# Ameek94/BOBE

Measured on AMD Instinct MI355X. Metric: GP fit+acquisition cycles/sec at N=4096 d=8, 65536 cands; Cholesky GF/s, higher is better.
Workload: dtype f64

## Files before the change

bobe_amd/_lib.py:

```python
from __future__ import annotations

import ctypes as C
import os
from typing import Optional

import numpy as np

_HERE = os.path.dirname(os.path.abspath(__file__))
LIB_PATH = os.path.join(_HERE, "libbobe_gp.so")

BOBE_OK = 0
BOBE_NOT_PD = 1
MAX_MLL_SLOTS = 8
PROF = {"potf2": 1, "trsm": 2, "syrk": 3, "trtri": 4, "lauum": 5, "trimul": 6, "cross": 7, "kxx": 8, "crossvv": 9, "kxc": 10}

c_double_p = C.POINTER(C.c_double)
c_int64_p = C.POINTER(C.c_int64)


class BobeLibraryError(RuntimeError):
    pass


SIGNATURES = [
# ... 59 lines not shown
    ("bobe_mgpu_world", C.c_int, []),
    ("bobe_mgpu_rank", C.c_int, []),
    ("bobe_mgpu_finalize", None, []),
    ("bobe_mgpu_wip_sweep", C.c_int, [C.c_void_p, C.c_void_p, C.c_int64, C.c_int64, C.c_void_p, C.c_int64, C.c_double,
                                      C.c_void_p, C.c_void_p, C.c_void_p, C.c_void_p,
                                      c_int64_p, c_double_p, c_int64_p, c_double_p]),
    ("bobe_mgpu_best_fit", C.c_int, [C.c_double, C.c_void_p, C.c_int, c_double_p, C.c_void_p]),
    ("bobe_gp_npoints", C.c_int64, [C.c_void_p]),
    ("bobe_debug_gemm", C.c_int, [C.c_int, C.c_int, C.c_int, C.c_int64, C.c_int64, C.c_int64, C.c_void_p, C.c_int64,
                                  C.c_void_p, C.c_int64, C.c_void_p, C.c_int64]),
    ("bobe_debug_kinv", C.c_int, [C.c_void_p, C.c_void_p]),
    ("bobe_debug_linv", C.c_int, [C.c_void_p, C.c_void_p]),
    ("bobe_debug_time_potrf", C.c_int, [C.c_void_p, C.c_int, c_double_p]),
    ("bobe_debug_time_potrf_batch", C.c_int, [C.c_void_p, C.c_int, C.c_int, c_double_p]),
    ("bobe_debug_time_potrf_lockstep", C.c_int, [C.c_void_p, C.c_int, C.c_int, c_double_p]),
    ("bobe_gp_set_chunk", C.c_int, [C.c_void_p, C.c_int64]),
    ("bobe_gp_profile_select", C.c_int, [C.c_void_p, C.c_int]),
    ("bobe_gp_profile_read", C.c_int, [C.c_void_p, c_double_p, c_int64_p]),
    ("bobe_debug_mfma_peak", C.c_int, [C.c_int, C.c_int, c_double_p]),
    ("bobe_debug_wave_sums", C.c_int, [C.c_int, C.c_int, C.c_void_p, C.c_void_p]),
]

_lib: Optional[C.CDLL] = None


def load() -> C.CDLL:
    global _lib
    if _lib is not None:
        return _lib
    if not os.path.exists(LIB_PATH):
# ... 42 lines not shown
```

bobe_amd/csrc/gp_abi.hip:

```cpp
#include "gp_handle.hpp"

#include "kernels_common.hpp"

#include <dlfcn.h>
#include <rccl/rccl.h>

using namespace bobe;

namespace bobe {
thread_local std::string g_err;
}

namespace {

template <int LA, int LB>
__global__ __launch_bounds__(256, 2) void k_debug_gemm(const double* __restrict__ A, int64_t lda,
                                                    const double* __restrict__ B, int64_t ldb, double* __restrict__ C,
                                                    int64_t ldc, int64_t K) {
  extern __shared__ double smem[];
  v4d acc[4][4];
  acc_zero(acc);
  gemm_tile<LA, LB>(acc, A, lda, (int64_t)blockIdx.y * TILE, B, ldb, (int64_t)blockIdx.x * TILE, 0, K, smem);
  store_tile(acc, C, ldc, (int64_t)blockIdx.y * TILE, (int64_t)blockIdx.x * TILE, 1.0, 0.0);
}
// ... 513 lines not shown
  API_BEGIN
  NEED(g && ms && reps >= 1 && B >= 1 && B <= BOBE_MAX_MLL_SLOTS, "bad argument");
  *ms = g->time_potrf_batch(B, reps);
  return BOBE_OK;
  API_END
}

int bobe_debug_time_potrf_lockstep(bobe_gp_t* g, int B, int reps, double* ms) {
  API_BEGIN
  NEED(g && ms && reps >= 1 && B >= 1 && B <= BOBE_MAX_MLL_SLOTS, "bad argument");
  *ms = g->time_potrf_lockstep(B, reps);
  return BOBE_OK;
  API_END
}

int bobe_gp_profile_select(bobe_gp_t* g, int tag) {
  API_BEGIN
  NEED(g, "gp is NULL");
  g->use();
  g->sync();
  g->prof_tag = tag;
  g->prof_used = 0;
  return BOBE_OK;
  API_END
}

int bobe_gp_profile_read(bobe_gp_t* g, double* total_ms, int64_t* launches) {
  API_BEGIN
  NEED(g && total_ms && launches, "NULL argument");
  g->use();
// ... 306 lines not shown
```

bobe_amd/csrc/gp_consumers.hip:

```cpp
#include "gp_handle.hpp"

#include "consumer_kernels.hpp"

using namespace bobe;

namespace bobe {
void configure_consumer_kernels() {
  static bool done[64] = {false};
  int dev = 0;
  HIPCHK(hipGetDevice(&dev));
  if (dev < 0 || dev >= 64 || done[dev]) return;
#define BIG(KE, DC)                                         \
  allow_big_lds((k_hmc_run<KE, DC>), CHAIN_LDS_BYTES);      \
  allow_big_lds((k_rwalk<KE, DC>), CHAIN_LDS_BYTES)
  BIG(0, 8); BIG(0, 16); BIG(0, 32); BIG(1, 8); BIG(1, 16); BIG(1, 32);
#undef BIG
  done[dev] = true;
}
}

void bobe_gp::set_gate(const double* sv, int64_t n_sv, const double* dual, double intercept, double gamma, double threshold,
                       double minus_inf) {
  use();
  sync();
// ... 289 lines not shown
      for (auto& v : dg) v += hk.noise;
      HIPCHK(hipMemcpy2D(out, (size_t)(nB + 1) * sizeof(double), dg.data(), sizeof(double), sizeof(double), (size_t)nA,
                         hipMemcpyHostToDevice));
    }
  }
}

void bobe_gp::clone_from(bobe_gp& src) {
  if (this == &src) return;
  if (d != src.d || kern != src.kern || device != src.device)
    throw Err(BOBE_ERR_ARG, "clone needs handles of the same kernel, dimension and device");
  if (!src.have_data) throw Err(BOBE_ERR_STATE, "source holds no data");
  src.use();
  src.sync();
  sync();
  N = src.N;
  hyp = src.hyp;
  pivot_ulp = src.pivot_ulp;
  refine_kappa = src.refine_kappa;
  solve_block = src.solve_block;
  solve_panel = src.solve_panel;
  solve_chunk = src.solve_chunk;
  refine_v = src.factored && src.refine_v;
  if (Np != src.Np) {
    Np = src.Np;
    nb = src.nb;
    alloc_for_n();
  }
  const size_t mat = (size_t)src.Np * src.Np * sizeof(double), vec = (size_t)src.Np * sizeof(double);
  X.ensure((size_t)(src.Np + TILE) * src.d * sizeof(double));
// ... 66 lines not shown
```

bobe_amd/csrc/gp_factor.hip:

```cpp
#include "gp_handle.hpp"

#include <chrono>

#include "chol_kernels.hpp"

using namespace bobe;

namespace bobe {

constexpr int SYRK32_BK = 128, SYRK64_BK = 16;
constexpr int SYRK32_SMEM = gemm_smem_doubles_exact<KC, KC, 32, 32, SYRK32_BK>() * 8 / 2;
constexpr int SYRK64_SMEM = gemm_smem_doubles_exact<KC, KC, 64, 64, SYRK64_BK>() * 8;

void configure_factor_kernels() {
  static bool done[64] = {false};
  int dev = 0;
  HIPCHK(hipGetDevice(&dev));
  if (dev < 0 || dev >= 64 || done[dev]) return;
  allow_big_lds(k_potf2<true>, POTF2_SMEM_BYTES);
  allow_big_lds(k_potf2<false>, POTF2_SMEM_BYTES);
  allow_big_lds(k_trti_diag, POTF2_SMEM_BYTES);
  allow_big_lds(k_trsm_panel, TRSM_SMEM_BYTES);
  allow_big_lds((k_chol_panel<false, 3>), POTF2_SMEM_BYTES);
  allow_big_lds((k_chol_panel<false, 4>), POTF2_SMEM_BYTES);
// ... 13 lines not shown
  allow_big_lds(k_lauum_grad<0, 32, 64>, GEMM64_SMEM_BYTES);
  allow_big_lds(k_lauum_grad<1, 8, 64>, GEMM64_SMEM_BYTES);
  allow_big_lds(k_lauum_grad<1, 16, 64>, GEMM64_SMEM_BYTES);
  allow_big_lds(k_lauum_grad<1, 32, 64>, GEMM64_SMEM_BYTES);
  allow_big_lds(k_lauum_grad<0, 8, 128>, GEMM_SMEM_BYTES);
  allow_big_lds(k_lauum_grad<0, 16, 128>, GEMM_SMEM_BYTES);
  allow_big_lds(k_lauum_grad<0, 32, 128>, GEMM_SMEM_BYTES);
  allow_big_lds(k_lauum_grad<1, 8, 128>, GEMM_SMEM_BYTES);
  allow_big_lds(k_lauum_grad<1, 16, 128>, GEMM_SMEM_BYTES);
  allow_big_lds(k_lauum_grad<1, 32, 128>, GEMM_SMEM_BYTES);
  done[dev] = true;
}

const Tuning& tuning() {
  static Tuning t = [] {
    Tuning v{512, 600, 300, 1, BOBE_MAX_MLL_SLOTS, 2048, 1, 1, false, false};
    auto geti = [](const char* name, int& dst) {
      const char* e = std::getenv(name);
      if (e) dst = std::atoi(e);
      return e != nullptr;
    };
    geti("BOBE_SYRK32_BELOW", v.syrk32_below);
    geti("BOBE_TRTRI64", v.trtri64_below);
    geti("BOBE_PAIR_MIN", v.pair_min);
    geti("BOBE_LOCKSTEP_MIN_N", v.lockstep_min_n);
    v.mll_slots_set = geti("BOBE_MLL_SLOTS", v.mll_slots);
    geti("BOBE_GRAPH_MAX_N", v.graph_max_n);
    geti("BOBE_XCD_SHARES", v.xcd_shares);
    geti("BOBE_FILL", v.fill);
    v.trace = std::getenv("BOBE_TRACE") != nullptr;
    return v;
  }();
  return t;
}

double default_refine_kappa() {
  static const double v = [] {
    const char* e = std::getenv("BOBE_REFINE_KAPPA");
    return e ? std::atof(e) : 1e6;
  }();
  return v;
}

int default_solve_block() {
  static const int v = [] {
// ... 79 lines not shown
  alpha.ensure(vec);
  w.ensure(vec);
  alpha2.ensure(vec);
  w2.ensure(vec);
  XsT.ensure((size_t)d * vec);
  XsT2.ensure((size_t)d * vec);
  const int64_t pw = Np > chunk ? Np : chunk;
  part.ensure((size_t)nb * pw * sizeof(double));
  gpart.ensure((size_t)(2 * nb) * (2 * nb + 1) / 2 * (MAX_D + 1) * sizeof(double));
  res.ensure(128 * sizeof(double));
  info.ensure(sizeof(int));
  flags.ensure((size_t)nb * sizeof(int));
  diag.ensure((size_t)nb * TILE * TILE * sizeof(double));
  build_probs();
  build_plans();
}

void bobe_gp::scale(const double* in, int64_t n, int64_t npad, const Hyper& h, double* out, int64_t ldo,
                    const Hyper* hdev, int B, int64_t bsO, int* info_reset) {
  hipLaunchKernelGGL(k_scale_coords, dim3((unsigned)((npad + 255) / 256), (unsigned)B), dim3(256), 0, stream, in, n, npad,
                     h, out, ldo, hdev, bsO, info_reset);
  LAUNCH_CHECK();
}

#define KM_LAUNCH(KE, SQ, DC, grid, ...)                                                                 \
  do {                                                                                                   \
    if (h.d == DC)                                                                                       \
      hipLaunchKernelGGL((k_kernel_matrix<KE, SQ, DC, true>), grid, dim3(256), 0, stream, __VA_ARGS__);  \
    else                                                                                                 \
      hipLaunchKernelGGL((k_kernel_matrix<KE, SQ, DC, false>), grid, dim3(256), 0, stream, __VA_ARGS__); \
// ... 402 lines not shown
  factor_into(h, XsT2.d(), A2.d(), Linv2.d(), w2.d(), alpha2.d(), hdev);
  if (want_grad) {
    const int dcap = d <= 8 ? 8 : (d <= 16 ? 16 : 32);
    const int ntiles = lauum(h, Linv2.d(), alpha2.d(), XsT2.d(), nullptr, dcap, hdev, nullptr, 1, 0, 0, 0, 0, Tmp.d(), 0);
    hipLaunchKernelGGL(k_mll_grad_reduce, dim3(d + 2), dim3(256), 0, stream, (const double*)gpart.d(), ntiles, dcap + 1, d,
                       dcap, res.d(), (const double*)w2.d(), (const double*)A2.d(), Np, Np, (const int*)info.p);
  } else {
    hipLaunchKernelGGL(k_mll_terms, dim3(1), dim3(256), 0, stream, (const double*)w2.d(), (const double*)A2.d(), Np, Np,
                       res.d(), (int64_t)0, (int64_t)0, (int64_t)0, (const int*)info.p);
  }
  LAUNCH_CHECK();
  HIPCHK(hipMemcpyAsync(h_res, res.p, 102 * sizeof(double), hipMemcpyDeviceToHost, stream));
}

void bobe_gp::mll_enqueue(const Hyper& h, bool want_grad) {
  const Tuning& tu = tuning();
  h_res[110] = pivot_floor(h);
  if (!in_slot || N > tu.graph_max_n || prof_tag != 0) {
    mll_enqueue_body(h, want_grad, nullptr);
    return;
  }
  if (!eg.h_hyp) HIPCHK(hipHostMalloc(reinterpret_cast<void**>(&eg.h_hyp), sizeof(Hyper), hipHostMallocDefault));
  eg.hyp_dev.ensure(sizeof(Hyper));
  const int w = want_grad ? 1 : 0;
  const std::array<const void*, 16> sig = eval_signature();
  if (!eg.exec[w] || eg.sig[w] != sig) {
    if (eg.exec[w]) {
      (void)hipGraphExecDestroy(eg.exec[w]);
      eg.exec[w] = nullptr;
    }
// ... 10 lines not shown
    const hipError_t ie = hipGraphInstantiate(&eg.exec[w], graph, nullptr, nullptr, 0);
    (void)hipGraphDestroy(graph);
    if (ie != hipSuccess) {
      eg.exec[w] = nullptr;
      HIPCHK(ie);
    }
    eg.sig[w] = sig;
  }
  *eg.h_hyp = h;
  HIPCHK(hipGraphLaunch(eg.exec[w], stream));
}

int bobe_gp::slot_collect(Slot& sl, double* mll, double* grad) {
  HIPCHK(hipStreamSynchronize(sl.stream));
  const double* hr = sl.h_res;
  int inf;
  std::memcpy(&inf, hr + 100, sizeof(int));
  if (inf != 0x7f7f7f7f || !pivots_resolved(hr[101], hr[110])) {
    *mll = std::nan("");
    if (grad)
      for (int j = 0; j <= d; ++j) grad[j] = std::nan("");
    g_err = not_pd_text(inf, hr[101]);
    return BOBE_NOT_PD;
  }
  *mll = -0.5 * hr[0] - hr[1] - 0.5 * (double)N * std::log(2.0 * M_PI);
  if (grad)
    for (int j = 0; j <= d; ++j) grad[j] = hr[2 + j];
  return BOBE_OK;
}

int bobe_gp::mll_collect(double* mll, double* grad) {
  sync();
  int inf;
  std::memcpy(&inf, h_res + 100, sizeof(int));
  if (inf != 0x7f7f7f7f || !pivots_resolved(h_res[101], h_res[110])) {
    *mll = std::nan("");
    if (grad)
      for (int j = 0; j <= d; ++j) grad[j] = std::nan("");
    g_err = not_pd_text(inf, h_res[101]);
    return BOBE_NOT_PD;
  }
  *mll = -0.5 * h_res[0] - h_res[1] - 0.5 * (double)N * std::log(2.0 * M_PI);
  if (grad)
    for (int j = 0; j <= d; ++j) grad[j] = h_res[2 + j];
  return BOBE_OK;
}

void bobe_gp::ensure_batch(int B) {
  if (!bw.h_hyp) {
    HIPCHK(hipHostMalloc(reinterpret_cast<void**>(&bw.h_hyp), BOBE_MAX_MLL_SLOTS * sizeof(Hyper), hipHostMallocDefault));
    HIPCHK(hipHostMalloc(reinterpret_cast<void**>(&bw.h_res), BOBE_MAX_MLL_SLOTS * 128 * sizeof(double), hipHostMallocDefault));
  }
  const size_t mat = (size_t)Np * Np * sizeof(double), vec = (size_t)Np * sizeof(double);
  const size_t nB = (size_t)B;
  bw.A.ensure(nB * mat); bw.Linv.ensure(nB * mat); bw.Tmp.ensure(nB * mat);
  bw.XsT.ensure(nB * d * vec); bw.w.ensure(nB * vec); bw.alpha.ensure(nB * vec);
  bw.part.ensure(nB * nb * vec);
  bw.gpart.ensure(nB * (size_t)gpart_stride() * sizeof(double));
  bw.res.ensure(nB * 128 * sizeof(double));
  bw.info.ensure(BOBE_MAX_MLL_SLOTS * sizeof(int));
  bw.diag.ensure(nB * (size_t)nb * TILE * TILE * sizeof(double));
  bw.hyp.ensure(BOBE_MAX_MLL_SLOTS * sizeof(Hyper));
  bw.cap = std::max(bw.cap, B);
  bw.Np = Np;
  (void)chol_plan(B, fill_pays(B));
}

void bobe_gp::mll_lockstep_enqueue(int B, const Hyper* hs, bool want_grad) {
  ensure_batch(B);
  const int64_t mat = Np * Np, vec = Np, xs = (int64_t)d * Np, prt = (int64_t)nb * Np, gps = gpart_stride();
  for (int b = 0; b < B; ++b) bw.h_hyp[b] = hs[b];
  HIPCHK(hipMemcpyAsync(bw.hyp.p, bw.h_hyp, (size_t)B * sizeof(Hyper), hipMemcpyHostToDevice, stream));
  const Hyper* hdev = static_cast<const Hyper*>(bw.hyp.p);
  int* inf = static_cast<int*>(bw.info.p);
  scale(X.d(), N, Np, hs[0], bw.XsT.d(), Np, hdev, B, xs, inf);
  assemble_kxx(hs[0], bw.XsT.d(), bw.A.d(), hdev, B, xs, mat);
  potrf(bw.A.d(), bw.Linv.d(), inf, B, mat, mat, bw.diag.d(), true);
  trtri(bw.A.d(), bw.Linv.d(), bw.Tmp.d(), B, mat, mat, mat);
  solve_alpha(bw.Linv.d(), bw.w.d(), bw.alpha.d(), bw.part.d(), B, mat, vec, prt);
  if (want_grad) {
    const int dcap = d <= 8 ? 8 : (d <= 16 ? 16 : 32);
    const int ntiles = lauum(hs[0], bw.Linv.d(), bw.alpha.d(), bw.XsT.d(), nullptr, dcap, hdev, bw.gpart.d(), B, mat, vec,
                             xs, gps, bw.Tmp.d(), mat);
    hipLaunchKernelGGL(k_mll_grad_reduce, dim3(d + 2, B), dim3(256), 0, stream, (const double*)bw.gpart.d(), ntiles, dcap + 1,
                       d, dcap, bw.res.d(), (const double*)bw.w.d(), (const double*)bw.A.d(), Np, Np, (const int*)inf, gps,
                       (int64_t)128, vec, mat);
  } else {
    hipLaunchKernelGGL(k_mll_terms, dim3(B), dim3(256), 0, stream, (const double*)bw.w.d(), (const double*)bw.A.d(), Np, Np,
                       bw.res.d(), vec, mat, (int64_t)128, (const int*)inf);
  }
  LAUNCH_CHECK();
  HIPCHK(hipMemcpyAsync(bw.h_res, bw.res.p, (size_t)B * 128 * sizeof(double), hipMemcpyDeviceToHost, stream));
}

int bobe_gp::mll_lockstep_collect(int B, double* mll, double* grad, int* status) {
  sync();
  int worst = BOBE_OK;
  for (int b = 0; b < B; ++b) {
    const double* hr = bw.h_res + (size_t)b * 128;
    double* gb = grad ? grad + (size_t)b * (d + 1) : nullptr;
    int st = BOBE_OK;
    int inf_b;
    std::memcpy(&inf_b, hr + 100, sizeof(int));
    if (inf_b != 0x7f7f7f7f || !pivots_resolved(hr[101], pivot_floor(bw.h_hyp[b]))) {
      mll[b] = std::nan("");
      if (gb)
        for (int j = 0; j <= d; ++j) gb[j] = std::nan("");
      g_err = not_pd_text(inf_b, hr[101]);
      st = BOBE_NOT_PD;
      worst = st;
    } else {
      mll[b] = -0.5 * hr[0] - hr[1] - 0.5 * (double)N * std::log(2.0 * M_PI);
      if (gb)
        for (int j = 0; j <= d; ++j) gb[j] = hr[2 + j];
    }
    if (status) status[b] = st;
  }
  return worst;
}

void bobe_gp::fill(double* p, int64_t n, double v) {
  hipLaunchKernelGGL(k_fill, dim3((unsigned)((n + 255) / 256)), dim3(256), 0, stream, p, n, v);
}

void bobe_gp::set_data(const double* Xin, const double* ys, int64_t n) {
  use();
  sync();
  const int64_t np_new = round_up(n, TILE);
  N = n;
  if (np_new != Np) {
    Np = np_new;
    nb = (int)(Np / TILE);
    alloc_for_n();
  }
  X.ensure((size_t)(Np + TILE) * d * sizeof(double));
  HIPCHK(hipMemcpyAsync(X.p, Xin, (size_t)N * d * sizeof(double),
                        is_device_ptr(Xin) ? hipMemcpyDeviceToDevice : hipMemcpyHostToDevice, stream));
  HIPCHK(hipMemsetAsync(y.p, 0, (size_t)Np * sizeof(double), stream));
  HIPCHK(hipMemcpyAsync(y.p, ys, (size_t)N * sizeof(double),
                        is_device_ptr(ys) ? hipMemcpyDeviceToDevice : hipMemcpyHostToDevice, stream));
  sync();
  have_data = true;
  factored = false;
  forget_z();
}

int bobe_gp::factor_state() {
  use();
  factor_into(hyp, XsT.d(), A.d(), Linv.d(), w.d(), alpha.d());
  hipLaunchKernelGGL(k_mll_terms, dim3(1), dim3(256), 0, stream, (const double*)w.d(), (const double*)A.d(), Np, Np, res.d(),
                     (int64_t)0, (int64_t)0, (int64_t)0, (const int*)info.p);
  LAUNCH_CHECK();
  HIPCHK(hipMemcpyAsync(h_res, res.p, 102 * sizeof(double), hipMemcpyDeviceToHost, stream));
  sync();
  int inf;
  std::memcpy(&inf, h_res + 100, sizeof(int));
  const double min_diag = h_res[101];
  factored = true;
  forget_z();
  not_pd = (inf != 0x7f7f7f7f) || !pivots_resolved(min_diag, pivot_floor(hyp));
  if (not_pd) {
    const double nan = std::nan("");
    fill(A.d(), Np * Np, nan);
    fill(Linv.d(), Np * Np, nan);
    fill(alpha.d(), Np, nan);
    LAUNCH_CHECK();
    sync();
    g_err = not_pd_text(inf, min_diag);
    refine_v = false;
    return BOBE_NOT_PD;
  }
  decide_refinement(min_diag);
// ... 135 lines not shown
}

void bobe_gp::get_chol(double* L, double* alpha_out) {
  if (!factored) throw Err(BOBE_ERR_STATE, "call bobe_gp_factor first");
  use();
  if (L) copy_out_matrix(A.d(), L, not_pd ? 0 : 1);
  if (alpha_out)
    HIPCHK(hipMemcpyAsync(alpha_out, alpha.p, (size_t)N * sizeof(double),
                          is_device_ptr(alpha_out) ? hipMemcpyDeviceToDevice : hipMemcpyDeviceToHost, stream));
  sync();
}

void bobe_gp::set_chol(const double* L, const double* alpha_in) {
  if (!have_data) throw Err(BOBE_ERR_STATE, "call bobe_gp_set_data first");
  use();
  const double* l_in = fetch(L, (size_t)N * N, kout);
  hipLaunchKernelGGL(k_load_padded_lower, dim3((unsigned)((Np + 255) / 256), (unsigned)Np), dim3(256), 0, stream, l_in, N,
                     A.d(), Np, Np);
  HIPCHK(hipMemsetAsync(alpha.p, 0, (size_t)Np * sizeof(double), stream));
  HIPCHK(hipMemcpyAsync(alpha.p, alpha_in, (size_t)N * sizeof(double),
                        is_device_ptr(alpha_in) ? hipMemcpyDeviceToDevice : hipMemcpyHostToDevice, stream));
  scale(X.d(), N, Np, hyp, XsT.d(), Np);
  for (int k = 0; k < nb; ++k)
    hipLaunchKernelGGL(k_potf2<false>, dim3(1), dim3(256), POTF2_SMEM_BYTES, stream, A.d(), Np, Linv.d(), Np, k,
                       static_cast<int*>(info.p));
  LAUNCH_CHECK();
  trtri(A.d(), Linv.d(), Tmp.d());
  const double min_diag = min_pivot_root();
  factored = true;
  forget_z();
// ... 1 lines not shown
  decide_refinement(min_diag);
}

double bobe_gp::min_pivot_root() {
  hipLaunchKernelGGL(k_mll_terms, dim3(1), dim3(256), 0, stream, (const double*)nullptr, (const double*)A.d(), Np, Np, res.d(),
                     (int64_t)0, (int64_t)0, (int64_t)0, (const int*)nullptr);
  LAUNCH_CHECK();
  HIPCHK(hipMemcpyAsync(h_res, res.p, 102 * sizeof(double), hipMemcpyDeviceToHost, stream));
  sync();
  return h_res[101];
}

void bobe_gp::size_workspace(int64_t n) {
  if (have_data && n != N) throw Err(BOBE_ERR_STATE, "the handle holds training data of another size (use a data-less handle)");
  if (have_data) return;
  const int64_t np_new = round_up(n, TILE);
  N = n;
  if (np_new != Np) {
    Np = np_new;
    nb = (int)(Np / TILE);
    alloc_for_n();
  }
}

int bobe_gp::mll_from_k(const double* K, int64_t n, const double* yv, double* mll) {
  use();
  sync();
  size_workspace(n);
  const double* k_in = fetch(K, (size_t)n * n, kout);
  hipLaunchKernelGGL(k_load_padded_lower, dim3((unsigned)((Np + 255) / 256), (unsigned)Np), dim3(256), 0, stream, k_in, n,
                     A2.d(), Np, Np, 1);
  HIPCHK(hipMemsetAsync(w.p, 0, (size_t)Np * sizeof(double), stream));
  HIPCHK(hipMemcpyAsync(w.p, yv, (size_t)n * sizeof(double),
                        is_device_ptr(yv) ? hipMemcpyDeviceToDevice : hipMemcpyHostToDevice, stream));
  HIPCHK(hipMemsetAsync(info.p, 0x7f, sizeof(int), stream));
  potrf(A2.d(), Linv2.d(), static_cast<int*>(info.p), 1, 0, 0, nullptr, true);
  trtri(A2.d(), Linv2.d(), Tmp.d());
  solve_alpha(Linv2.d(), w2.d(), alpha2.d(), part.d(), 1, 0, 0, 0, w.d(), 0);
  hipLaunchKernelGGL(k_mll_terms, dim3(1), dim3(256), 0, stream, (const double*)w2.d(), (const double*)A2.d(), Np, Np, res.d(),
                     (int64_t)0, (int64_t)0, (int64_t)0, (const int*)info.p);
  LAUNCH_CHECK();
  HIPCHK(hipMemcpyAsync(h_res, res.p, 102 * sizeof(double), hipMemcpyDeviceToHost, stream));
  sync();
  int inf;
  std::memcpy(&inf, h_res + 100, sizeof(int));
  if (inf != 0x7f7f7f7f || !(h_res[101] > 0.0)) {
    *mll = std::nan("");
    g_err = not_pd_text(inf, h_res[101]);
    return BOBE_NOT_PD;
  }
  *mll = -0.5 * h_res[0] - h_res[1] - 0.5 * (double)n * std::log(2.0 * M_PI);
  return BOBE_OK;
}

void bobe_gp::chol_row_update(const double* L, int64_t n, const double* k, double k_self, double* v, double* diag_out) {
  use();
  sync();
  size_workspace(n);
  const double* l_in = fetch(L, (size_t)n * n, kout);
  hipLaunchKernelGGL(k_load_padded_lower, dim3((unsigned)((Np + 255) / 256), (unsigned)Np), dim3(256), 0, stream, l_in, n,
                     A2.d(), Np, Np, 0);
  HIPCHK(hipMemsetAsync(w.p, 0, (size_t)Np * sizeof(double), stream));
  HIPCHK(hipMemcpyAsync(w.p, k, (size_t)n * sizeof(double),
                        is_device_ptr(k) ? hipMemcpyDeviceToDevice : hipMemcpyHostToDevice, stream));
  for (int kb = 0; kb < nb; ++kb)
    hipLaunchKernelGGL(k_potf2<false>, dim3(1), dim3(256), POTF2_SMEM_BYTES, stream, A2.d(), Np, Linv2.d(), Np, kb,
                       static_cast<int*>(info.p));
  LAUNCH_CHECK();
  trtri(A2.d(), Linv2.d(), Tmp.d());
  hipLaunchKernelGGL(k_gemv_lower, dim3((unsigned)(Np / 4), 1u), dim3(256), 0, stream, (const double*)Linv2.d(), Np, Np,
                     (const double*)w.d(), w2.d(), (int64_t)0, (int64_t)0, (int64_t)0);
  hipLaunchKernelGGL(k_mll_terms, dim3(1), dim3(256), 0, stream, (const double*)w2.d(), (const double*)A2.d(), Np, Np, res.d(),
                     (int64_t)0, (int64_t)0, (int64_t)0, (const int*)nullptr);
// ... 30 lines not shown
    (void)hipEventDestroy(e0);
    (void)hipEventDestroy(e1);
  }
  double ms() {
    HIPCHK(hipEventSynchronize(e1));
    float t = 0.f;
    HIPCHK(hipEventElapsedTime(&t, e0, e1));
    return t;
  }
};
}

double bobe_gp::time_potrf(int reps) {
  if (!have_data) throw Err(BOBE_ERR_STATE, "call bobe_gp_set_data first");
  use();
  EventPair ev;
  double total = 0.0;
  scale(X.d(), N, Np, hyp, XsT2.d(), Np);
  for (int r = -1; r < reps; ++r) {
    assemble_kxx(hyp, XsT2.d(), A2.d());
    HIPCHK(hipMemsetAsync(info.p, 0x7f, sizeof(int), stream));
    HIPCHK(hipEventRecord(ev.e0, stream));
    potrf(A2.d(), Linv2.d(), static_cast<int*>(info.p));
    HIPCHK(hipEventRecord(ev.e1, stream));
    const double t = ev.ms();
    if (r >= 0) total += t;
  }
  return total / reps;
}

double bobe_gp::time_potrf_batch(int B, int reps) {
  if (!have_data) throw Err(BOBE_ERR_STATE, "call bobe_gp_set_data first");
  use();
  ensure_slots(B);
  const std::vector<hipStream_t>& sts = slot_stream_set();
  EventPair ev;
  std::vector<hipEvent_t> done(B);
  for (auto& e : done) HIPCHK(hipEventCreateWithFlags(&e, hipEventDisableTiming));
  double total = 0.0;
  for (int r = -1; r < reps; ++r) {
    for (int i = 0; i < B; ++i) {
      Slot& sl = *slots[i];
      scale(X.d(), N, Np, hyp, sl.XsT2.d(), Np);
      assemble_kxx(hyp, sl.XsT2.d(), sl.A2.d());
      HIPCHK(hipMemsetAsync(sl.info.p, 0x7f, sizeof(int), stream));
    }
    HIPCHK(hipEventRecord(ev.e0, stream));
    for (int i = 0; i < B; ++i) {
// ... 10 lines not shown
      swap_slot(sl);
      HIPCHK(hipEventRecord(done[i], sl.stream));
      HIPCHK(hipStreamWaitEvent(stream, done[i], 0));
    }
    HIPCHK(hipEventRecord(ev.e1, stream));
    const double t = ev.ms();
    if (r >= 0) total += t;
  }
  for (auto& e : done) (void)hipEventDestroy(e);
  return total / reps;
}

double bobe_gp::time_potrf_lockstep(int B, int reps) {
  if (!have_data) throw Err(BOBE_ERR_STATE, "call bobe_gp_set_data first");
  use();
  ensure_batch(B);
  const int64_t mat = Np * Np, xs = (int64_t)d * Np;
  for (int b = 0; b < B; ++b) bw.h_hyp[b] = hyp;
  HIPCHK(hipMemcpyAsync(bw.hyp.p, bw.h_hyp, (size_t)B * sizeof(Hyper), hipMemcpyHostToDevice, stream));
  const Hyper* hdev = static_cast<const Hyper*>(bw.hyp.p);
  EventPair ev;
  double total = 0.0;
  scale(X.d(), N, Np, hyp, bw.XsT.d(), Np, hdev, B, xs);
  for (int r = -1; r < reps; ++r) {
    assemble_kxx(hyp, bw.XsT.d(), bw.A.d(), hdev, B, xs, mat);
    HIPCHK(hipMemsetAsync(bw.info.p, 0x7f, (size_t)B * sizeof(int), stream));
    HIPCHK(hipEventRecord(ev.e0, stream));
    potrf(bw.A.d(), bw.Linv.d(), static_cast<int*>(bw.info.p), B, mat, mat, bw.diag.d());
    HIPCHK(hipEventRecord(ev.e1, stream));
    const double t = ev.ms();
// ... 5 lines not shown
```

bobe_amd/csrc/gp_handle.hpp:

```cpp
#pragma once
#include "../../include/bobe_gp.h"

#include <hip/hip_runtime.h>

#include <algorithm>
#include <array>
#include <climits>
#include <cmath>
#include <cstdio>
#include <cstdlib>
#include <cstring>
#include <map>
#include <mutex>
#include <stdexcept>
#include <string>
#include <vector>

#include "gemm_f64.hpp"
#include "gp_types.hpp"

namespace bobe {

struct Err : std::runtime_error {
  int code;
// ... 50 lines not shown
}
inline bool pivots_resolved(double min_diag, double floor) { return min_diag * min_diag >= floor; }
double default_pivot_floor_ulp();
double default_refine_kappa();
int default_solve_block();
int default_solve_panel();
int64_t default_solve_chunk();

template <typename K>
void allow_big_lds(K kernel, int bytes) {
  HIPCHK(hipFuncSetAttribute(reinterpret_cast<const void*>(kernel), hipFuncAttributeMaxDynamicSharedMemorySize, bytes));
}

struct Tuning {
  int syrk32_below, trtri64_below, pair_min, lockstep_min_n, mll_slots, graph_max_n, xcd_shares, fill;
  bool mll_slots_set, trace;
};
const Tuning& tuning();

constexpr int LAUUM64_BELOW = 1200;
constexpr int FILL_NEAR = 2;
constexpr int FILL_CHUNK = 3;
constexpr int FILL_SLACK = 16;
constexpr int FILL_PHASE = 1024;

struct TileGrid { int grid, per; };
inline TileGrid tile_grid(int ntiles) {
  if (!tuning().xcd_shares || ntiles < 256) return {ntiles, 0};
  const int per = (ntiles + 7) / 8;
  return {8 * per, per};
}

void configure_factor_kernels();
void configure_sweep_kernels();
void configure_consumer_kernels();

struct Depth { int first, count, nblocks; };

}

struct bobe_gp {
  typedef bobe::DBuf DBuf;
  typedef bobe::Hyper Hyper;
  int device = 0;
  int kern = 0;
  int d = 0;
  hipStream_t stream = nullptr;
  bool own_stream = false;
  int64_t N = 0, Np = 0;
  int nb = 0;
  Hyper hyp;
  double pivot_ulp = bobe::default_pivot_floor_ulp();
  double pivot_floor(const Hyper& h) const { return bobe::pivot_floor(h, pivot_ulp); }
  bool have_data = false, factored = false, not_pd = false;
  double refine_kappa = bobe::default_refine_kappa();
  bool refine_v = false;
  int solve_block = bobe::default_solve_block();
  int solve_panel = bobe::default_solve_panel();
  int64_t solve_chunk = bobe::default_solve_chunk();
  void decide_refinement(double min_diag);
  void solve_v(double* B, int64_t ldb, int64_t ncp, double* V, int64_t ldv, double* qp, int64_t ldq);
  std::vector<double> z_seen;
  int64_t z_seen_m = -1;
  bool wz_ready = false;
  void forget_z() { z_seen_m = -1; wz_ready = false; }
  int64_t chunk = 8192;
// ... 48 lines not shown
  int panel_strips(int B, int rr) const;

  struct EvalGraph {
    hipGraphExec_t exec[2] = {nullptr, nullptr};
    std::array<const void*, 16> sig[2] = {};
    Hyper* h_hyp = nullptr;
    DBuf hyp_dev;
  };
  struct Slot {
    hipStream_t stream = nullptr;
    DBuf XsT2, A2, Linv2, Tmp, alpha2, w2, part, gpart, res, info, flags, diag;
    EvalGraph eg;
    double* h_res = nullptr;
    hipEvent_t ev = nullptr;
    bool busy = false, want_grad = false;
  };
  EvalGraph eg;
  std::array<const void*, 16> eval_signature() const {
    return {XsT2.p, A2.p, Linv2.p, Tmp.p, w2.p, alpha2.p, part.p, gpart.p, res.p, info.p, X.p, y.p, probs.p,
            static_cast<const void*>(h_res), reinterpret_cast<const void*>(static_cast<uintptr_t>(N)),
            static_cast<const void*>(stream)};
  }
  void mll_enqueue_body(const Hyper& h, bool want_grad, const Hyper* hdev);
  std::vector<Slot*> slots;
  std::vector<hipStream_t> slot_streams;
  const std::vector<hipStream_t>& slot_stream_set();
  hipEvent_t ev_batch = nullptr;
  bool in_slot = false;
  void swap_slot(Slot& s) {
    std::swap(stream, s.stream);
    std::swap(XsT2, s.XsT2); std::swap(A2, s.A2); std::swap(Linv2, s.Linv2); std::swap(Tmp, s.Tmp);
    std::swap(alpha2, s.alpha2); std::swap(w2, s.w2); std::swap(part, s.part); std::swap(gpart, s.gpart);
    std::swap(res, s.res); std::swap(info, s.info); std::swap(flags, s.flags); std::swap(diag, s.diag);
    std::swap(h_res, s.h_res);
    std::swap(eg, s.eg);
    in_slot = !in_slot;
  }
  struct BatchWs {
    int cap = 0;
    int64_t Np = 0;
    DBuf A, Linv, Tmp, XsT, w, alpha, part, gpart, res, info, hyp, diag;
    Hyper* h_hyp = nullptr;
    double* h_res = nullptr;
  } bw;
  int64_t gpart_stride() const { return (int64_t)(2 * nb) * (2 * nb + 1) / 2 * (bobe::MAX_D + 1); }
  void ensure_batch(int B);
  void mll_lockstep_enqueue(int B, const Hyper* hs, bool want_grad);
  int mll_lockstep_collect(int B, double* mll, double* grad, int* status);
  std::mutex submit_mutex;
  void ensure_slots(int n);
  void mll_enqueue(const Hyper& h, bool want_grad);
  int slot_collect(Slot& sl, double* mll, double* grad);
  int mll_collect(double* mll, double* grad);
  int mll_batch(int64_t B, const double* ls, const double* kvar, double* mll, double* grad, int* status);
  void mll_submit(int slot, const double* ls, double kvar, int want_grad);
  int mll_wait(int slot, double* mll, double* grad);

  int prof_tag = 0;
  std::vector<std::pair<hipEvent_t, hipEvent_t>> prof_events;
  size_t prof_used = 0;
  void prof_begin(int tag) {
    if (tag != prof_tag) return;
    if (prof_used == prof_events.size()) {
      hipEvent_t a, b;
      HIPCHK(hipEventCreate(&a));
      HIPCHK(hipEventCreate(&b));
// ... 49 lines not shown
  int aside_first = 1 << 30;
  const double* aside_dg = nullptr;
  void trtri(double* a, double* linv, double* tmp, int B = 1, int64_t bsA = 0, int64_t bsL = 0, int64_t bsT = 0);
  int lauum(const Hyper& h, const double* linv, const double* al, const double* xst, double* kinv_out, int dcap,
            const Hyper* hdev = nullptr, double* gp_out = nullptr, int B = 1, int64_t bsL = 0, int64_t bsV = 0,
            int64_t bsX = 0, int64_t bsP = 0, double* scratch = nullptr, int64_t bsS = 0);
  void solve_alpha(const double* linv, double* wv, double* al, double* prt, int B = 1, int64_t bsL = 0, int64_t bsV = 0,
                   int64_t bsP = 0, const double* rhs = nullptr, int64_t bsY = 0);
  void factor_into(const Hyper& h, double* xst, double* a, double* linv, double* wv, double* al,
                   const Hyper* hdev = nullptr);
  std::string not_pd_text(int inf, double min_diag) const;
  void size_workspace(int64_t n);
  int mll_from_k(const double* K, int64_t n, const double* yv, double* mll);
  void chol_row_update(const double* L, int64_t n, const double* k, double k_self, double* v, double* diag_out);
  int factor_state();
  void copy_out_matrix(const double* src, double* dst, int lower_only);
  void get_chol(double* L, double* alpha_out);
  void set_chol(const double* L, const double* alpha_in);
  double min_pivot_root();
  void kinv_debug(double* Kinv);
  double time_potrf(int reps);
  double time_potrf_batch(int B, int reps);
  double time_potrf_lockstep(int B, int reps);
  void fill(double* p, int64_t n, double v);

  void prepare_z(const double* Z, int64_t M, int64_t Mp, bool need_w);
  void sweep(const double* cand, int64_t C, const double* Z, int64_t M, double y_std, double* wipv, double* wipstd,
             double* mean, double* var, int policy, int64_t* argmin_v, double* min_v, int64_t* argmin_s, double* min_s,
             double* fantasy_out, bool gated = false);
  void wip_grad(const double* cand, int64_t C, const double* Z, int64_t M, double y_std, double* wipv, double* wipstd,
// ... 18 lines not shown
```

bobe_amd/csrc/gp_sweep.hip:

```cpp
#include "gp_handle.hpp"

#include "sweep_kernels.hpp"

using namespace bobe;

namespace bobe {
void configure_sweep_kernels() {
  static bool done[64] = {false};
  int dev = 0;
  HIPCHK(hipGetDevice(&dev));
  if (dev < 0 || dev >= 64 || done[dev]) return;
  allow_big_lds(k_trimul, GEMM_SMEM_BYTES);
  allow_big_lds(k_trimul_t, GEMM_SMEM_BYTES);
  allow_big_lds(k_trimul_v64, GEMM64_SMEM_BYTES);
  allow_big_lds(k_trimul_t64, GEMM64_SMEM_BYTES);
  allow_big_lds(k_blk_step, GEMM_SMEM_BYTES);
  allow_big_lds(k_cross_vv<128>, GEMM_SMEM_BYTES);
  allow_big_lds(k_cross_vv<64>, GEMM64_SMEM_BYTES);
  done[dev] = true;
}
}

void bobe_gp::decide_refinement(double min_diag) {
  const double piv = min_diag * min_diag;
// ... 461 lines not shown
  out_finish(mean, C, o_mean);
  out_finish(var, C, o_var);
  out_finish(dmean, (size_t)C * d, o_wipv);
  out_finish(dvar, (size_t)C * d, o_wipstd);
  sync();
}

int bobe_gp::append(const double* X_new, int64_t b, const double* y_all) {
  if (!factored || not_pd) throw Err(BOBE_ERR_STATE, "append needs a positive-definite factorised state");
  use();
  sync();
  const int64_t N0 = N, N1 = N0 + b, Np0 = Np, Np1 = round_up(N1, TILE);
  factored = false;
  have_data = false;
  forget_z();
  DBuf nx, oa, ol;
  try {
  const bool xnew_on_device = is_device_ptr(X_new);
  {
    const size_t need = (size_t)N1 * d * sizeof(double);
    if (X.bytes < need) {
      nx.ensure((size_t)(Np1 + TILE) * d * sizeof(double));
      HIPCHK(hipMemcpyAsync(nx.p, X.p, (size_t)N0 * d * sizeof(double), hipMemcpyDeviceToDevice, stream));
      sync();
      std::swap(X, nx);
      nx.release();
    }
    HIPCHK(hipMemcpyAsync(X.d() + N0 * d, X_new, (size_t)b * d * sizeof(double),
                          xnew_on_device ? hipMemcpyDeviceToDevice : hipMemcpyHostToDevice, stream));
  }
// ... 112 lines not shown
```

bobe_amd/csrc/kernels_common.hpp:

```cpp
#pragma once
#include "gemm_f64.hpp"
#include "gp_types.hpp"

namespace bobe {

constexpr double SQRT5 = 2.23606797749978969641;
constexpr double NOISE_FLOOR = 1e-12;

template <int KERN>
__device__ __forceinline__ double kern_eval(double r2, double kvar) {
  if (KERN == 0) {
    return kvar * exp(-0.5 * r2);
  } else if (KERN == 2) {
    return r2;
  } else {
    const double dd = sqrt(r2 < 1e-30 ? 1e-30 : r2);
    const double e = exp(-SQRT5 * dd);
    const double poly = 1.0 + dd * (SQRT5 + (dd * 5.0) / 3.0);
    return kvar * poly * e;
  }
}

template <int KERN>
__device__ __forceinline__ double kern_grad_factor(double r2, double kvar, double kval) {
// ... 275 lines not shown
  partial += slot * bsP;
  res += slot * bsR;
  const int j = blockIdx.x;
  const int src = (j == d) ? dcap : j;
  double s = 0.0;
  for (int q = threadIdx.x; q < ntiles; q += 64) s += partial[(int64_t)q * stride + src];
  s = wave_sum(s);
  if (threadIdx.x == 0) res[2 + j] = 0.5 * s;
}

static __global__ void k_fill(double* __restrict__ p, int64_t n, double v) {
  const int64_t i = (int64_t)blockIdx.x * blockDim.x + threadIdx.x;
  if (i < n) p[i] = v;
}

static __global__ void k_copy2d(const double* __restrict__ src, int64_t lds, double* __restrict__ dst, int64_t ldd, int64_t rows,
                         int64_t cols, int lower_only) {
  const int64_t j = (int64_t)blockIdx.x * blockDim.x + threadIdx.x;
  const int64_t i = blockIdx.y;
  if (i < rows && j < cols) dst[i * ldd + j] = (lower_only && j > i) ? 0.0 : src[i * lds + j];
}

static __global__ void k_load_padded_lower(const double* __restrict__ src, int64_t n, double* __restrict__ dst, int64_t ld,
                                    int64_t np, int whole = 0) {
  const int64_t j = (int64_t)blockIdx.x * blockDim.x + threadIdx.x;
  const int64_t i = blockIdx.y;
  if (i >= np || j >= np) return;
  double v;
  if (i < n && j < n) v = (j <= i || whole) ? src[i * n + j] : 0.0;
  else v = (i == j) ? 1.0 : 0.0;
// ... 5 lines not shown
```

include/bobe_gp.h:

```cpp
#ifndef BOBE_GP_H
#define BOBE_GP_H
#include <stdint.h>

#ifdef __cplusplus
extern "C" {
#endif

typedef struct bobe_gp bobe_gp_t;

#define BOBE_OK 0
#define BOBE_NOT_PD 1
#define BOBE_ERR_ARG (-1)
#define BOBE_ERR_HIP (-2)
#define BOBE_ERR_STATE (-3)

#define BOBE_KERNEL_RBF 0
#define BOBE_KERNEL_MATERN 1

const char* bobe_version(void);
const char* bobe_last_error(void);
int bobe_device_count(void);

int bobe_gp_create(bobe_gp_t** out, int device, int kernel, int d);
void bobe_gp_destroy(bobe_gp_t* gp);
// ... 88 lines not shown
void bobe_mgpu_finalize(void);
int bobe_mgpu_wip_sweep(bobe_gp_t* gp, const double* cand_shard, int64_t C, int64_t global_offset, const double* Z,
                        int64_t M, double y_std, double* wipv, double* wipstd, double* mean, double* var,
                        int64_t* argmin_v, double* min_v, int64_t* argmin_s, double* min_s);
int bobe_mgpu_best_fit(double mll, const double* theta, int n, double* best_mll, double* best_theta);

int64_t bobe_gp_npoints(bobe_gp_t* gp);

int bobe_debug_gemm(int device, int layoutA, int layoutB, int64_t M, int64_t N, int64_t K, const double* A,
                    int64_t lda, const double* B, int64_t ldb, double* C, int64_t ldc);
int bobe_debug_kinv(bobe_gp_t* gp, double* Kinv);
int bobe_debug_linv(bobe_gp_t* gp, double* Linv);
int bobe_debug_time_potrf(bobe_gp_t* gp, int reps, double* ms);
int bobe_debug_time_potrf_batch(bobe_gp_t* gp, int B, int reps, double* ms);
int bobe_debug_time_potrf_lockstep(bobe_gp_t* gp, int B, int reps, double* ms);
#define BOBE_PROF_POTF2 1
#define BOBE_PROF_TRSM 2
#define BOBE_PROF_SYRK 3
#define BOBE_PROF_TRTRI 4
#define BOBE_PROF_LAUUM 5
#define BOBE_PROF_TRIMUL 6
#define BOBE_PROF_CROSS 7
#define BOBE_PROF_KXX 8
#define BOBE_PROF_CROSSVV 9
#define BOBE_PROF_KXC 10
int bobe_gp_profile_select(bobe_gp_t* gp, int kernel_class);
int bobe_gp_profile_read(bobe_gp_t* gp, double* total_ms, int64_t* launches);
int bobe_debug_mfma_peak(int device, int waves_per_simd, double* tflops);
int bobe_debug_wave_sums(int device, int D, const double* in, double* out);
int bobe_gp_set_chunk(bobe_gp_t* gp, int64_t chunk);
// ... 7 lines not shown
```

Measured before the change: 17.60.

## Reuse Cholesky factor from a matching MLL evaluation instead of refactoring

Tags every MLL evaluation workspace (single, slot, lockstep batch) with the hyperparameters, data generation and padded size. When factor_state runs with hyperparameters that exactly match a completed evaluation, it copies that evaluation's factor, inverse, alpha, w and scaled inputs with a single copy kernel instead of recomputing the Cholesky. Invalidation hooks are added to every data mutation path. This adds bookkeeping and the risk of stale reuse if any invalidation path is missed.

```diff
diff --git a/bobe_amd/_lib.py b/bobe_amd/_lib.py
--- a/bobe_amd/_lib.py
+++ b/bobe_amd/_lib.py
@@ -97,6 +97,7 @@
     ("bobe_debug_time_potrf", C.c_int, [C.c_void_p, C.c_int, c_double_p]),
     ("bobe_debug_time_potrf_batch", C.c_int, [C.c_void_p, C.c_int, C.c_int, c_double_p]),
     ("bobe_debug_time_potrf_lockstep", C.c_int, [C.c_void_p, C.c_int, C.c_int, c_double_p]),
+    ("bobe_debug_factor_source", C.c_int, [C.c_void_p]),
     ("bobe_gp_set_chunk", C.c_int, [C.c_void_p, C.c_int64]),
     ("bobe_gp_profile_select", C.c_int, [C.c_void_p, C.c_int]),
     ("bobe_gp_profile_read", C.c_int, [C.c_void_p, c_double_p, c_int64_p]),
diff --git a/bobe_amd/csrc/gp_abi.hip b/bobe_amd/csrc/gp_abi.hip
--- a/bobe_amd/csrc/gp_abi.hip
+++ b/bobe_amd/csrc/gp_abi.hip
@@ -551,6 +551,8 @@
   API_END
 }
 
+int bobe_debug_factor_source(bobe_gp_t* g) { return g ? g->factor_source : -1; }
+
 int bobe_gp_profile_select(bobe_gp_t* g, int tag) {
   API_BEGIN
   NEED(g, "gp is NULL");
diff --git a/bobe_amd/csrc/gp_consumers.hip b/bobe_amd/csrc/gp_consumers.hip
--- a/bobe_amd/csrc/gp_consumers.hip
+++ b/bobe_amd/csrc/gp_consumers.hip
@@ -327,6 +327,9 @@
   src.use();
   src.sync();
   sync();
+  ++data_gen;
+  forget_evals();
+  factor_source = -1;
   N = src.N;
   hyp = src.hyp;
   pivot_ulp = src.pivot_ulp;
diff --git a/bobe_amd/csrc/gp_factor.hip b/bobe_amd/csrc/gp_factor.hip
--- a/bobe_amd/csrc/gp_factor.hip
+++ b/bobe_amd/csrc/gp_factor.hip
@@ -51,7 +51,7 @@
 
 const Tuning& tuning() {
   static Tuning t = [] {
-    Tuning v{512, 600, 300, 1, BOBE_MAX_MLL_SLOTS, 2048, 1, 1, false, false};
+    Tuning v{512, 600, 300, 1, BOBE_MAX_MLL_SLOTS, 2048, 1, 1, false, false, true};
     auto geti = [](const char* name, int& dst) {
       const char* e = std::getenv(name);
       if (e) dst = std::atoi(e);
@@ -66,6 +66,9 @@
     geti("BOBE_XCD_SHARES", v.xcd_shares);
     geti("BOBE_FILL", v.fill);
     v.trace = std::getenv("BOBE_TRACE") != nullptr;
+    int reuse = 1;
+    geti("BOBE_FACTOR_REUSE", reuse);
+    v.factor_reuse = reuse != 0;
     return v;
   }();
   return t;
@@ -175,6 +178,7 @@
   diag.ensure((size_t)nb * TILE * TILE * sizeof(double));
   build_probs();
   build_plans();
+  forget_evals();
 }
 
 void bobe_gp::scale(const double* in, int64_t n, int64_t npad, const Hyper& h, double* out, int64_t ldo,
@@ -607,6 +611,12 @@
 }
 
 void bobe_gp::mll_enqueue(const Hyper& h, bool want_grad) {
+  tag2.clear();
+  mll_enqueue_pipeline(h, want_grad);
+  tag2.arm(h, data_gen, Np);
+}
+
+void bobe_gp::mll_enqueue_pipeline(const Hyper& h, bool want_grad) {
   const Tuning& tu = tuning();
   h_res[110] = pivot_floor(h);
   if (!in_slot || N > tu.graph_max_n || prof_tag != 0) {
@@ -647,6 +657,7 @@
 int bobe_gp::slot_collect(Slot& sl, double* mll, double* grad) {
   HIPCHK(hipStreamSynchronize(sl.stream));
   const double* hr = sl.h_res;
+  sl.tag.collected(hr);
   int inf;
   std::memcpy(&inf, hr + 100, sizeof(int));
   if (inf != 0x7f7f7f7f || !pivots_resolved(hr[101], hr[110])) {
@@ -664,6 +675,7 @@
 
 int bobe_gp::mll_collect(double* mll, double* grad) {
   sync();
+  tag2.collected(h_res);
   int inf;
   std::memcpy(&inf, h_res + 100, sizeof(int));
   if (inf != 0x7f7f7f7f || !pivots_resolved(h_res[101], h_res[110])) {
@@ -686,6 +698,8 @@
   }
   const size_t mat = (size_t)Np * Np * sizeof(double), vec = (size_t)Np * sizeof(double);
   const size_t nB = (size_t)B;
+  if (B > bw.cap || Np != bw.Np)
+    for (bobe::EvalTag& t : bw.tag) t.clear();
   bw.A.ensure(nB * mat); bw.Linv.ensure(nB * mat); bw.Tmp.ensure(nB * mat);
   bw.XsT.ensure(nB * d * vec); bw.w.ensure(nB * vec); bw.alpha.ensure(nB * vec);
   bw.part.ensure(nB * nb * vec);
@@ -702,6 +716,7 @@
 void bobe_gp::mll_lockstep_enqueue(int B, const Hyper* hs, bool want_grad) {
   ensure_batch(B);
   const int64_t mat = Np * Np, vec = Np, xs = (int64_t)d * Np, prt = (int64_t)nb * Np, gps = gpart_stride();
+  for (int b = 0; b < B; ++b) bw.tag[b].clear();
   for (int b = 0; b < B; ++b) bw.h_hyp[b] = hs[b];
   HIPCHK(hipMemcpyAsync(bw.hyp.p, bw.h_hyp, (size_t)B * sizeof(Hyper), hipMemcpyHostToDevice, stream));
   const Hyper* hdev = static_cast<const Hyper*>(bw.hyp.p);
@@ -724,6 +739,7 @@
   }
   LAUNCH_CHECK();
   HIPCHK(hipMemcpyAsync(bw.h_res, bw.res.p, (size_t)B * 128 * sizeof(double), hipMemcpyDeviceToHost, stream));
+  for (int b = 0; b < B; ++b) bw.tag[b].arm(hs[b], data_gen, Np);
 }
 
 int bobe_gp::mll_lockstep_collect(int B, double* mll, double* grad, int* status) {
@@ -731,6 +747,7 @@
   int worst = BOBE_OK;
   for (int b = 0; b < B; ++b) {
     const double* hr = bw.h_res + (size_t)b * 128;
+    bw.tag[b].collected(hr);
     double* gb = grad ? grad + (size_t)b * (d + 1) : nullptr;
     int st = BOBE_OK;
     int inf_b;
@@ -759,6 +776,8 @@
 void bobe_gp::set_data(const double* Xin, const double* ys, int64_t n) {
   use();
   sync();
+  ++data_gen;
+  forget_evals();
   const int64_t np_new = round_up(n, TILE);
   N = n;
   if (np_new != Np) {
@@ -778,17 +797,74 @@
   forget_z();
 }
 
+void bobe_gp::forget_evals() {
+  tag2.clear();
+  for (Slot* sl : slots) sl->tag.clear();
+  for (bobe::EvalTag& t : bw.tag) t.clear();
+}
+
+const bobe::EvalTag* bobe_gp::adopt_factor() {
+  if (!tuning().factor_reuse || in_slot) return nullptr;
+  auto match = [&](const bobe::EvalTag& t) { return t.valid && t.gen == data_gen && t.Np == Np && bobe::same_hyper(t.h, hyp); };
+  const size_t mat = (size_t)Np * Np, vec = (size_t)Np, xs = (size_t)d * Np;
+  const bobe::EvalTag* tag = nullptr;
+  const double *sA = nullptr, *sL = nullptr, *sal = nullptr, *sw = nullptr, *sx = nullptr;
+  int src = 0;
+  if (bw.Np == Np)
+    for (int b = 0; b < bw.cap && b < BOBE_MAX_MLL_SLOTS && !tag; ++b) {
+      const size_t b1 = (size_t)b + 1;
+      if (!match(bw.tag[b]) || bw.A.bytes < b1 * mat * 8 || bw.Linv.bytes < b1 * mat * 8 || bw.alpha.bytes < b1 * vec * 8 ||
+          bw.w.bytes < b1 * vec * 8 || bw.XsT.bytes < b1 * xs * 8)
+        continue;
+      tag = &bw.tag[b];
+      sA = bw.A.d() + b * mat; sL = bw.Linv.d() + b * mat; sal = bw.alpha.d() + b * vec; sw = bw.w.d() + b * vec;
+      sx = bw.XsT.d() + b * xs;
+      src = 1;
+    }
+  if (!tag) {
+    std::lock_guard<std::mutex> lock(submit_mutex);
+    for (Slot* sl : slots)
+      if (!sl->busy && match(sl->tag)) {
+        tag = &sl->tag;
+        sA = sl->A2.d(); sL = sl->Linv2.d(); sal = sl->alpha2.d(); sw = sl->w2.d(); sx = sl->XsT2.d();
+        src = 2;
+        break;
+      }
+  }
+  if (!tag && match(tag2)) {
+    tag = &tag2;
+    sA = A2.d(); sL = Linv2.d(); sal = alpha2.d(); sw = w2.d(); sx = XsT2.d();
+    src = 3;
+  }
+  if (!tag) return nullptr;
+  const int vgroups = (int)std::min<int64_t>(64, ((int64_t)xs + 255) / 256);
+  hipLaunchKernelGGL(k_copy_factor, dim3((unsigned)(nb * (nb + 1) + vgroups)), dim3(256), 0, stream, sA, A.d(), sL, Linv.d(),
+                     nb, sal, alpha.d(), sw, w.d(), sx, XsT.d(), Np, (int64_t)xs);
+  LAUNCH_CHECK();
+  sync();
+  factor_source = src;
+  if (tuning().trace) std::fprintf(stderr, "[bobe] factor: adopted the factor of an evaluation (source %d)\n", src);
+  return tag;
+}
+
 int bobe_gp::factor_state() {
   use();
-  factor_into(hyp, XsT.d(), A.d(), Linv.d(), w.d(), alpha.d());
-  hipLaunchKernelGGL(k_mll_terms, dim3(1), dim3(256), 0, stream, (const double*)w.d(), (const double*)A.d(), Np, Np, res.d(),
-                     (int64_t)0, (int64_t)0, (int64_t)0, (const int*)info.p);
-  LAUNCH_CHECK();
-  HIPCHK(hipMemcpyAsync(h_res, res.p, 102 * sizeof(double), hipMemcpyDeviceToHost, stream));
-  sync();
   int inf;
-  std::memcpy(&inf, h_res + 100, sizeof(int));
-  const double min_diag = h_res[101];
+  double min_diag;
+  if (const bobe::EvalTag* t = adopt_factor()) {
+    inf = t->info;
+    min_diag = t->min_diag;
+  } else {
+    factor_into(hyp, XsT.d(), A.d(), Linv.d(), w.d(), alpha.d());
+    hipLaunchKernelGGL(k_mll_terms, dim3(1), dim3(256), 0, stream, (const double*)w.d(), (const double*)A.d(), Np, Np, res.d(),
+                       (int64_t)0, (int64_t)0, (int64_t)0, (const int*)info.p);
+    LAUNCH_CHECK();
+    HIPCHK(hipMemcpyAsync(h_res, res.p, 102 * sizeof(double), hipMemcpyDeviceToHost, stream));
+    sync();
+    std::memcpy(&inf, h_res + 100, sizeof(int));
+    min_diag = h_res[101];
+    factor_source = 0;
+  }
   factored = true;
   forget_z();
   not_pd = (inf != 0x7f7f7f7f) || !pivots_resolved(min_diag, pivot_floor(hyp));
@@ -954,6 +1030,9 @@
 void bobe_gp::set_chol(const double* L, const double* alpha_in) {
   if (!have_data) throw Err(BOBE_ERR_STATE, "call bobe_gp_set_data first");
   use();
+  ++data_gen;
+  forget_evals();
+  factor_source = -1;
   const double* l_in = fetch(L, (size_t)N * N, kout);
   hipLaunchKernelGGL(k_load_padded_lower, dim3((unsigned)((Np + 255) / 256), (unsigned)Np), dim3(256), 0, stream, l_in, N,
                      A.d(), Np, Np);
@@ -985,6 +1064,7 @@
 void bobe_gp::size_workspace(int64_t n) {
   if (have_data && n != N) throw Err(BOBE_ERR_STATE, "the handle holds training data of another size (use a data-less handle)");
   if (have_data) return;
+  ++data_gen;
   const int64_t np_new = round_up(n, TILE);
   N = n;
   if (np_new != Np) {
@@ -998,6 +1078,7 @@
   use();
   sync();
   size_workspace(n);
+  forget_evals();
   const double* k_in = fetch(K, (size_t)n * n, kout);
   hipLaunchKernelGGL(k_load_padded_lower, dim3((unsigned)((Np + 255) / 256), (unsigned)Np), dim3(256), 0, stream, k_in, n,
                      A2.d(), Np, Np, 1);
@@ -1028,6 +1109,7 @@
   use();
   sync();
   size_workspace(n);
+  forget_evals();
   const double* l_in = fetch(L, (size_t)n * n, kout);
   hipLaunchKernelGGL(k_load_padded_lower, dim3((unsigned)((Np + 255) / 256), (unsigned)Np), dim3(256), 0, stream, l_in, n,
                      A2.d(), Np, Np, 0);
@@ -1088,6 +1170,7 @@
 double bobe_gp::time_potrf(int reps) {
   if (!have_data) throw Err(BOBE_ERR_STATE, "call bobe_gp_set_data first");
   use();
+  forget_evals();
   EventPair ev;
   double total = 0.0;
   scale(X.d(), N, Np, hyp, XsT2.d(), Np);
@@ -1106,6 +1189,7 @@
 double bobe_gp::time_potrf_batch(int B, int reps) {
   if (!have_data) throw Err(BOBE_ERR_STATE, "call bobe_gp_set_data first");
   use();
+  forget_evals();
   ensure_slots(B);
   const std::vector<hipStream_t>& sts = slot_stream_set();
   EventPair ev;
@@ -1146,6 +1230,7 @@
 double bobe_gp::time_potrf_lockstep(int B, int reps) {
   if (!have_data) throw Err(BOBE_ERR_STATE, "call bobe_gp_set_data first");
   use();
+  forget_evals();
   ensure_batch(B);
   const int64_t mat = Np * Np, xs = (int64_t)d * Np;
   for (int b = 0; b < B; ++b) bw.h_hyp[b] = hyp;
diff --git a/bobe_amd/csrc/gp_handle.hpp b/bobe_amd/csrc/gp_handle.hpp
--- a/bobe_amd/csrc/gp_handle.hpp
+++ b/bobe_amd/csrc/gp_handle.hpp
@@ -88,7 +88,7 @@
 
 struct Tuning {
   int syrk32_below, trtri64_below, pair_min, lockstep_min_n, mll_slots, graph_max_n, xcd_shares, fill;
-  bool mll_slots_set, trace;
+  bool mll_slots_set, trace, factor_reuse;
 };
 const Tuning& tuning();
 
@@ -110,6 +110,36 @@
 void configure_consumer_kernels();
 
 struct Depth { int first, count, nblocks; };
+
+struct EvalTag {
+  bool pending = false;
+  bool valid = false;
+  Hyper h;
+  uint64_t gen = 0;
+  int64_t Np = 0;
+  int info = 0;
+  double min_diag = 0.0;
+  void arm(const Hyper& hh, uint64_t g, int64_t np) {
+    valid = false;
+    pending = true;
+    h = hh;
+    gen = g;
+    Np = np;
+  }
+  void collected(const double* hr) {
+    if (!pending) return;
+    pending = false;
+    valid = true;
+    std::memcpy(&info, hr + 100, sizeof(int));
+    min_diag = hr[101];
+  }
+  void clear() { pending = valid = false; }
+};
+inline bool same_hyper(const Hyper& a, const Hyper& b) {
+  if (a.d != b.d || a.kern != b.kern || a.d < 0 || a.d > MAX_D) return false;
+  return std::memcmp(a.ls, b.ls, (size_t)a.d * sizeof(double)) == 0 && std::memcmp(&a.kvar, &b.kvar, sizeof(double)) == 0 &&
+         std::memcmp(&a.noise, &b.noise, sizeof(double)) == 0;
+}
 
 }
 
@@ -124,6 +154,7 @@
   int64_t N = 0, Np = 0;
   int nb = 0;
   Hyper hyp;
+  uint64_t data_gen = 0;
   double pivot_ulp = bobe::default_pivot_floor_ulp();
   double pivot_floor(const Hyper& h) const { return bobe::pivot_floor(h, pivot_ulp); }
   bool have_data = false, factored = false, not_pd = false;
@@ -202,8 +233,10 @@
     double* h_res = nullptr;
     hipEvent_t ev = nullptr;
     bool busy = false, want_grad = false;
+    bobe::EvalTag tag;
   };
   EvalGraph eg;
+  bobe::EvalTag tag2;
   std::array<const void*, 16> eval_signature() const {
     return {XsT2.p, A2.p, Linv2.p, Tmp.p, w2.p, alpha2.p, part.p, gpart.p, res.p, info.p, X.p, y.p, probs.p,
             static_cast<const void*>(h_res), reinterpret_cast<const void*>(static_cast<uintptr_t>(N)),
@@ -222,6 +255,7 @@
     std::swap(res, s.res); std::swap(info, s.info); std::swap(flags, s.flags); std::swap(diag, s.diag);
     std::swap(h_res, s.h_res);
     std::swap(eg, s.eg);
+    std::swap(tag2, s.tag);
     in_slot = !in_slot;
   }
   struct BatchWs {
@@ -230,6 +264,7 @@
     DBuf A, Linv, Tmp, XsT, w, alpha, part, gpart, res, info, hyp, diag;
     Hyper* h_hyp = nullptr;
     double* h_res = nullptr;
+    std::array<bobe::EvalTag, BOBE_MAX_MLL_SLOTS> tag;
   } bw;
   int64_t gpart_stride() const { return (int64_t)(2 * nb) * (2 * nb + 1) / 2 * (bobe::MAX_D + 1); }
   void ensure_batch(int B);
@@ -238,6 +273,7 @@
   std::mutex submit_mutex;
   void ensure_slots(int n);
   void mll_enqueue(const Hyper& h, bool want_grad);
+  void mll_enqueue_pipeline(const Hyper& h, bool want_grad);
   int slot_collect(Slot& sl, double* mll, double* grad);
   int mll_collect(double* mll, double* grad);
   int mll_batch(int64_t B, const double* ls, const double* kvar, double* mll, double* grad, int* status);
@@ -317,6 +353,9 @@
   int mll_from_k(const double* K, int64_t n, const double* yv, double* mll);
   void chol_row_update(const double* L, int64_t n, const double* k, double k_self, double* v, double* diag_out);
   int factor_state();
+  void forget_evals();
+  const bobe::EvalTag* adopt_factor();
+  int factor_source = -1;
   void copy_out_matrix(const double* src, double* dst, int lower_only);
   void get_chol(double* L, double* alpha_out);
   void set_chol(const double* L, const double* alpha_in);
diff --git a/bobe_amd/csrc/gp_sweep.hip b/bobe_amd/csrc/gp_sweep.hip
--- a/bobe_amd/csrc/gp_sweep.hip
+++ b/bobe_amd/csrc/gp_sweep.hip
@@ -499,6 +499,9 @@
   factored = false;
   have_data = false;
   forget_z();
+  ++data_gen;
+  forget_evals();
+  factor_source = -1;
   DBuf nx, oa, ol;
   try {
   const bool xnew_on_device = is_device_ptr(X_new);
diff --git a/bobe_amd/csrc/kernels_common.hpp b/bobe_amd/csrc/kernels_common.hpp
--- a/bobe_amd/csrc/kernels_common.hpp
+++ b/bobe_amd/csrc/kernels_common.hpp
@@ -313,6 +313,37 @@
   if (i < n) p[i] = v;
 }
 
+static __global__ __launch_bounds__(256) void k_copy_factor(const double* __restrict__ sA, double* __restrict__ dA,
+                                                            const double* __restrict__ sL, double* __restrict__ dL, int nb,
+                                                            const double* __restrict__ sal, double* __restrict__ dal,
+                                                            const double* __restrict__ sw, double* __restrict__ dw,
+                                                            const double* __restrict__ sx, double* __restrict__ dx, int64_t np,
+                                                            int64_t nx) {
+  const int T = nb * (nb + 1) / 2;
+  int t = (int)blockIdx.x;
+  if (t < 2 * T) {
+    const double* s = t < T ? sA : sL;
+    double* o = t < T ? dA : dL;
+    t = t < T ? t : t - T;
+    int ti = (int)((sqrt(8.0 * t + 1.0) - 1.0) * 0.5);
+    while ((ti + 1) * (ti + 2) / 2 <= t) ++ti;
+    while (ti * (ti + 1) / 2 > t) --ti;
+    const int tj = t - ti * (ti + 1) / 2;
+    const int64_t base = (int64_t)ti * TILE * np + (int64_t)tj * TILE;
+    for (int e = threadIdx.x; e < TILE * TILE / 2; e += 256) {
+      const int64_t off = base + (int64_t)(e / (TILE / 2)) * np + 2 * (e % (TILE / 2));
+      *reinterpret_cast<double2*>(o + off) = *reinterpret_cast<const double2*>(s + off);
+    }
+    return;
+  }
+  const int64_t stride = (int64_t)(gridDim.x - 2 * T) * 256;
+  for (int64_t i = (int64_t)(blockIdx.x - 2 * T) * 256 + threadIdx.x; i < np; i += stride) {
+    dal[i] = sal[i];
+    dw[i] = sw[i];
+  }
+  for (int64_t i = (int64_t)(blockIdx.x - 2 * T) * 256 + threadIdx.x; i < nx; i += stride) dx[i] = sx[i];
+}
+
 static __global__ void k_copy2d(const double* __restrict__ src, int64_t lds, double* __restrict__ dst, int64_t ldd, int64_t rows,
                          int64_t cols, int lower_only) {
   const int64_t j = (int64_t)blockIdx.x * blockDim.x + threadIdx.x;
diff --git a/include/bobe_gp.h b/include/bobe_gp.h
--- a/include/bobe_gp.h
+++ b/include/bobe_gp.h
@@ -126,6 +126,7 @@
 int bobe_debug_time_potrf(bobe_gp_t* gp, int reps, double* ms);
 int bobe_debug_time_potrf_batch(bobe_gp_t* gp, int B, int reps, double* ms);
 int bobe_debug_time_potrf_lockstep(bobe_gp_t* gp, int B, int reps, double* ms);
+int bobe_debug_factor_source(bobe_gp_t* gp);
 #define BOBE_PROF_POTF2 1
 #define BOBE_PROF_TRSM 2
 #define BOBE_PROF_SYRK 3
```

Result: faster. 18.27, median of 6 (+3.8%).
